# samuelfneumann/RLControl

Hardware: AMD Instinct MI355X
Metric: gradient updates/sec/GPU (batch=100), Pendulum-shaped DDPG (higher is better)
Workload: dtype f32

## Files before the change

rlcontrol_amd/csrc/ddpg_mfma_kernel.h:

```cpp
#pragma once
#include "mfma_blocks.h"
#include "ddpg_rollout_device.h"

namespace {

using namespace mfb;

constexpr int NTW = 2;
constexpr int NT16 = 16;
constexpr int MSTRIDE = mask_stride(NT16);
static_assert(MSTRIDE == 272, "mask stride of the 256-wide kernels");

struct Smem {
    lds_f32* hbuf;
    lds_u8* mask;
    lds_f32* part;
    lds_f32* wvec;
    lds_f32 *x, *x2, *a, *aout, *mu, *dz, *q, *y, *dq;
    lds_f64 *r, *g;
    lds_i64* idx;
    lds_i32* pool;
    lds_i32* dups;
    lds_f32x4* xbuf;
    lds_f32 *w1t, *w1o;
};

__host__ __device__ inline bool rlc_mfma_wide(const RlcDims& d) { return d.S > SMAX || d.A > 2; }

template <bool WIDE = false>
__host__ __device__ inline size_t smem_carve(const RlcDims& d, int MT, lds_u8* base, Smem* out) {
    size_t off = 0;
    auto take = [&](size_t bytes) {
        lds_u8* p = base + off;
        off += (bytes + 15) & ~(size_t)15;
        return p;
    };
    const int MB = MT * 16, A = d.A, LDH = ldh_for(d.H1);
    constexpr bool wide = WIDE;
    const int XL = wide ? xld_for(d.S) : SMAX;
    Smem L;
    L.hbuf = (lds_f32*)take(sizeof(float) * (MB * LDH + 16));
    L.r = (lds_f64*)take(sizeof(double) * MB);
    L.g = (lds_f64*)take(sizeof(double) * MB);
    L.idx = (lds_i64*)take(sizeof(long long) * RLC_MAX_BATCH);
    L.mask = take((size_t)MB * MSTRIDE);
    static_assert(sizeof(float) * kWaves * 6 <= MSTRIDE, "the WIDE form's partials fit the mask rows");
    if constexpr (wide) L.part = (lds_f32*)L.mask;
    else L.part = (lds_f32*)take(sizeof(float) * kWaves * MB * A);
    L.wvec = (lds_f32*)take(sizeof(float) * A * 256);
    L.x = (lds_f32*)take(sizeof(float) * MB * XL);
    L.x2 = (lds_f32*)take(sizeof(float) * MB * XL);
    L.a = (lds_f32*)take(sizeof(float) * MB * A);
    L.aout = (lds_f32*)take(sizeof(float) * MB * A);
    L.mu = (lds_f32*)take(sizeof(float) * MB * A);
    if constexpr (wide) L.dz = L.a;
    else L.dz = (lds_f32*)take(sizeof(float) * MB * A);
    L.q = (lds_f32*)take(sizeof(float) * MB);
    L.y = (lds_f32*)take(sizeof(float) * MB);
    L.dq = (lds_f32*)take(sizeof(float) * MB);
    L.pool = (lds_i32*)take(sizeof(int) * 3 * RLC_MAX_BATCH);
    L.dups = (lds_i32*)take(sizeof(int) * 4);
    if constexpr (wide) {
        auto t13 = [](int n) { return (n + 15) >> 4 == 13; };
        if (t13(d.H1) || t13(d.HA) || t13(d.HC)) L.xbuf = (lds_f32x4*)take(sizeof(float) * 4 * 64 * (MT - (MT + 3) / 4));
        else L.xbuf = nullptr;
    } else {
        L.xbuf = (lds_f32x4*)take(sizeof(float) * 4 * 64 * (MT - (MT + 3) / 4));
    }
    L.w1t = L.w1o = nullptr;
    if (out) *out = L;
    return off;
}

template <int MT, int AD, bool FUSE, bool T4, bool WIDE = false>
__global__ __launch_bounds__(kThreads) void rlc_ddpg_update_mfma_kernel(RlcDev dv, int first_agent, int n_updates,
                                                                        int source, const long long* host_idx,
                                                                        int grad_taps, const RlcRollout* rollout,
                                                                        int q8_first) {
    extern __shared__ __attribute__((aligned(16))) unsigned char smem[];
    using U = Blk<MT, NTW, MSTRIDE, false, false, T4, WIDE>;
    static_assert(WIDE || AD <= 2, "more than two action columns: the WIDE form");
    static_assert(!(WIDE && T4), "the WIDE form has no tail-of-four units");
    constexpr int MB = U::MB;
    const RlcDims d = dv.d;
    U u;
    u.init_geometry();
    u.S = d.S; u.H1 = d.H1; u.B = d.B; u.LDH = ldh_for(d.H1);
    const int XL = WIDE ? xld_for(d.S) : SMAX;
    Smem L;
    smem_carve<WIDE>(d, MT, (lds_u8*)smem, &L);
    u.L.hbuf = L.hbuf; u.L.mask = L.mask; u.L.xbuf = L.xbuf;
    const int tid = u.tid, S = d.S, H1 = d.H1, HA = d.HA, HC = d.HC, B = d.B;
    const int agent = first_agent + blockIdx.x;
    constexpr bool fuse_fwd = FUSE;
    const bool sep = d.sep != 0;

    float* th = dv.theta + (size_t)agent * d.Ppad;
    float* tt = dv.theta_t + (size_t)agent * d.Ppad;
    float* m_a = dv.m_a + (size_t)agent * d.Ppad;
    float* v_a = dv.v_a + (size_t)agent * d.Ppad;
    float* m_c = dv.m_c + (size_t)agent * d.Ppad;
    float* v_c = dv.v_c + (size_t)agent * d.Ppad;
    float* pw = dv.pw + agent * 4;
    const float lr_a = dv.actor_lr[agent], lr_c = dv.critic_lr[agent], tau = dv.tau;
#ifdef RLC_STAMPS
    float* stamp_buf = grad_taps ? dv.tap_gc + (size_t)agent * d.Ppad : nullptr;
    float* tap_gc = nullptr;
    float* tap_ga = nullptr;
#else
    float* tap_gc = grad_taps ? dv.tap_gc + (size_t)agent * d.Ppad : nullptr;
    float* tap_ga = grad_taps ? dv.tap_ga + (size_t)agent * d.Ppad : nullptr;
#endif
    float amax[AD];
#pragma unroll
    for (int j = 0; j < AD; j++) amax[j] = dv.amax[j];

    for (int i = tid; i < MB * AD; i += kThreads) { L.a[i] = 0.f; L.aout[i] = 0.f; L.mu[i] = 0.f; L.dz[i] = 0.f; }
    for (int i = tid; i < MB * XL; i += kThreads) { L.x[i] = 0.f; L.x2[i] = 0.f; }
    for (int i = tid; i < MB; i += kThreads) { L.q[i] = 0.f; L.y[i] = 0.f; L.dq[i] = 0.f; }
    for (int i = tid; i < MB * MSTRIDE / 4; i += kThreads) reinterpret_cast<lds_u32*>(L.mask)[i] = 0u;
    if (tid < 16) L.hbuf[MB * u.LDH + tid] = 0.0f;
    __syncthreads();

    f32x4 acc[MT][NTW];
#ifdef RLC_STAMPS
    long long t_prev = clock64();
    int stamp_i = 0;
#define STAMP()                                                                                  \
    do {                                                                                         \
        if (tid == 0 && stamp_buf) { const long long t = clock64(); stamp_buf[stamp_i] += (float)(t - t_prev); t_prev = t; } \
        stamp_i++;                                                                               \
    } while (0)
    if (stamp_buf) for (int i = tid; i < 64; i += kThreads) stamp_buf[i] = 0.0f;
    const long long t_k0 = clock64(), w_k0 = wall_clock64();
    u.stamp_buf = stamp_buf;
    __syncthreads();
#else
#define STAMP() do {} while (0)
#endif

    for (int upd = 0; upd < n_updates; upd++) {
#ifdef RLC_STAMPS
        stamp_i = 0;
#endif
        asm volatile("" : "+v"(u.c), "+v"(u.g), "+s"(u.wave));
        if (rollout) {
            if (!rlc_train_step_device(rollout, agent, (float*)L.hbuf, upd == 0 ? q8_first : 0)) continue;
        }
        if (!(ablate(4) && upd > 0)) {
        u.sub_begin();
        const RlcRingMeta ring = dv.rep.ring[agent];
        if (source == RLC_SRC_REPLAY_DEVICE_SAMPLER) {
            const unsigned long long call = dv.rep.sample_ctr[agent];
            __syncthreads();
            u.sub_stamp(25);
            rlc_sample_distinct(ring.size, B, dv.rep.seed[agent], call, L.pool, L.idx, L.dups);
            if (tid == 0) dv.rep.sample_ctr[agent] = call + 1;
            u.sub_stamp(26);
        } else if (source == RLC_SRC_REPLAY_HOST_INDICES) {
            for (int b = tid; b < B; b += kThreads) L.idx[b] = host_idx[((size_t)blockIdx.x * n_updates + upd) * B + b];
        }
        __syncthreads();
        for (int b = tid; b < B; b += kThreads) {
            const float *ps, *pa, *ps2;
            if (source == RLC_SRC_STAGING) {
                const size_t slot = (size_t)agent * RLC_MAX_BATCH + b;
                ps = dv.rep.gs + slot * S; pa = dv.rep.ga + slot * AD; ps2 = dv.rep.gs2 + slot * S;
                L.r[b] = dv.rep.gr[slot]; L.g[b] = dv.rep.gg[slot];
            } else {
                const size_t slot = (size_t)agent * dv.rep.cap + ring_slot(ring, dv.rep.cap, L.idx[b]);
                ps = dv.rep.rs + slot * S; pa = dv.rep.ra + slot * AD; ps2 = dv.rep.rs2 + slot * S;
                L.r[b] = dv.rep.rr[slot]; L.g[b] = dv.rep.rg[slot];
            }
            for (int i = 0; i < S; i++) {
                L.x[b * XL + i] = clip_state_val(ps[i], dv.clip_state, dv.smin[i], dv.smax[i]);
                L.x2[b * XL + i] = clip_state_val(ps2[i], dv.clip_state, dv.smin[i], dv.smax[i]);
            }
#pragma unroll
            for (int j = 0; j < AD; j++) L.a[b * AD + j] = pa[j];
        }
        u.sub_stamp(27);
        }
        __syncthreads();
        STAMP();

        u.trunk(tt + d.oW1, tt + d.ob1, L.x2);
        __syncthreads();
        STAMP();
        f32x4 acc2[MT][NTW];
        if constexpr (fuse_fwd) u.fwd_gemm2(acc, acc2, tt + d.oWa2, tt + d.oWc2, HA, H1);
        else u.fwd_gemm(acc, tt + d.oWa2, HA, H1);
        u.template bias_relu<0>(acc, tt + d.oba2, HA);
        u.template row_dot<false, AD>(acc, HA, [&](int n, int j) { return tt[d.oWa3 + n * AD + j]; }, L.part);
        __syncthreads();
        STAMP();
        for (int i = tid; i < B * AD; i += kThreads) {
            const int b = i / AD, j = i % AD;
            L.aout[i] = tanhf(u.template part_sum<AD>(L.part, b, j) + tt[d.oba3 + j]) * amax[j];
        }
        __syncthreads();
        STAMP();
        if constexpr (fuse_fwd) {
#pragma unroll
            for (int mt = 0; mt < MT; mt++)
#pragma unroll
                for (int i = 0; i < NTW; i++) acc[mt][i] = acc2[mt][i];
        } else {
            if (sep) {
                u.trunk(tt + d.oWc1, tt + d.obc1, L.x2);
                __syncthreads();
            }
            u.fwd_gemm(acc, tt + d.oWc2, HC, H1);
        }
        u.template bias_relu<AD>(acc, tt + d.obc2, HC, L.aout, tt + d.oWc2, d.arow0);
        u.template row_dot<false, 1>(acc, HC, [&](int n, int) { return tt[d.oWc3 + n]; }, L.part);
        __syncthreads();
        STAMP();
        for (int b = tid; b < B; b += kThreads) {
            const float qt = u.template part_sum<1>(L.part, b, 0) + tt[d.obc3];
            const float y = (float)(L.r[b] + L.g[b] * (double)qt);
            L.y[b] = y;
            dv.tap_y[(size_t)agent * RLC_MAX_BATCH + b] = y;
        }
        __syncthreads();
        STAMP();

        u.trunk(th + d.oWc1, th + d.obc1, L.x);
        for (int n = tid; n < 256; n += kThreads) L.wvec[n] = n < HC ? th[d.oWc3 + n] : 0.0f;
        __syncthreads();
        STAMP();
        u.fwd_gemm(acc, th + d.oWc2, HC, H1);
        u.template bias_relu<AD>(acc, th + d.obc2, HC, L.a, th + d.oWc2, d.arow0);
        u.template row_dot<false, 1>(acc, HC, [&](int n, int) { return th[d.oWc3 + n]; }, L.part);
        __syncthreads();
        STAMP();
        for (int b = tid; b < B; b += kThreads) {
            const float q = u.template part_sum<1>(L.part, b, 0) + th[d.obc3];
            L.q[b] = q;
            dv.tap_q[(size_t)agent * RLC_MAX_BATCH + b] = q;
            L.dq[b] = 2.0f * (q - L.y[b]) / (float)B;
        }
        __syncthreads();
        STAMP();
        float g_wc3[NTW], g_bc2[NTW];
        {
            const int NT = (HC + 15) >> 4;
#pragma unroll
            for (int i = 0; i < NTW; i++) {
                const int t = u.tile_of(i);
                const int n = 16 * t + u.c;
                const float w3 = (t < NT && n < HC) ? L.wvec[n] : 0.0f;
                float s3 = 0.0f, s2 = 0.0f;
#pragma unroll
                for (int mt = 0; mt < MT; mt++) {
                    const f32x4 dq4 = *reinterpret_cast<const lds_f32x4*>(&L.dq[16 * mt + 4 * u.g]);
#pragma unroll
                    for (int r = 0; r < 4; r++) {
                        const float gv = acc[mt][i][r];
                        s3 += gv * dq4[r];
                        s2 += gv > 0.0f ? dq4[r] * w3 : 0.0f;
                    }
                }
                g_wc3[i] = col4_sum(s3);
                g_bc2[i] = col4_sum(s2);
            }
        }
        u.template store_masks<-2, true>(acc, HC);
        __syncthreads();
        STAMP();
        const float alpha_c = adam_alpha(lr_c, pw[2], pw[3]);
        u.template bwd_gemm<1, -2>(acc, th + d.oWc2, HC, H1, L.dq, L.wvec);
        __syncthreads();
        STAMP();
        u.trunk_grad_adam(acc, th, m_c, v_c, alpha_c, d.oWc1, d.obc1, tap_gc, sep ? tt : nullptr, tau, L.x);
        STAMP();
        u.template wgrad_adam<1, AD, -1>(L.dq, L.a, HC, th + d.oWc2, m_c + d.oWc2, v_c + d.oWc2, alpha_c,
                     tap_gc ? tap_gc + d.oWc2 : nullptr, tt + d.oWc2, tau, L.wvec);
        u.sub_begin();
        {
            const int NT = (HC + 15) >> 4;
#pragma unroll
            for (int i = 0; i < NTW; i++) {
                const int t = u.tile_of(i);
                const int n = 16 * t + u.c;
                if (t < NT && n < HC && u.g < 2) {
                    const int p = (u.g == 0) ? d.oWc3 + n : d.obc2 + n;
                    const float gr = (u.g == 0) ? g_wc3[i] : g_bc2[i];
                    float mm = m_c[p], vv = v_c[p];
                    const float o = tt[p];
                    const float nv = adam_step(th[p], gr, mm, vv, alpha_c);
                    m_c[p] = mm; v_c[p] = vv; th[p] = nv;
                    if (tap_gc) tap_gc[p] = gr;
                    tt[p] = o + tau * (nv - o);
                }
            }
            if (u.wave == 0) {
                float gr = 0.0f;
                for (int b = u.lane; b < MB; b += 64) gr += L.dq[b];
#pragma unroll
                for (int off = 32; off > 0; off >>= 1) gr += __shfl_xor(gr, off, 64);
                if (u.lane == 0) {
                    const int p = d.obc3;
                    float mm = m_c[p], vv = v_c[p];
                    const float o = tt[p];
                    const float nv = adam_step(th[p], gr, mm, vv, alpha_c);
                    m_c[p] = mm; v_c[p] = vv; th[p] = nv;
                    if (tap_gc) tap_gc[p] = gr;
                    tt[p] = o + tau * (nv - o);
                }
            }
        }
        u.sub_stamp(29);
        __syncthreads();
        u.sub_stamp(30);
        STAMP();
        if (tid == 0) { pw[2] *= 0.9f; pw[3] *= 0.999f; }

        u.trunk(th + d.oW1, th + d.ob1, L.x);
        for (int i = tid; i < AD * 256; i += kThreads) {
            const int j = i / 256, n = i % 256;
            L.wvec[i] = n < HA ? th[d.oWa3 + n * AD + j] : 0.0f;
        }
        __syncthreads();
        STAMP();
        f32x4 acc7[MT][NTW];
        if constexpr (fuse_fwd) u.fwd_gemm2(acc, acc7, th + d.oWa2, th + d.oWc2, HA, H1);
        else u.fwd_gemm(acc, th + d.oWa2, HA, H1);
        u.template bias_relu<0>(acc, th + d.oba2, HA);
        u.template row_dot<false, AD>(acc, HA, [&](int n, int j) { return th[d.oWa3 + n * AD + j]; }, L.part);
        if constexpr (!WIDE) u.template store_masks<-2, true>(acc, HA);
        __syncthreads();
        STAMP();
        for (int i = tid; i < B * AD; i += kThreads) {
            const int b = i / AD, j = i % AD;
            const float mu = tanhf(u.template part_sum<AD>(L.part, b, j) + th[d.oba3 + j]);
            L.mu[i] = mu;
            const float ao = mu * amax[j];
            L.aout[i] = ao;
            dv.tap_aout[(size_t)agent * RLC_MAX_BATCH * AD + i] = ao;
        }
        __syncthreads();
        STAMP();
        f32x4 h2acc[MT][NTW];
#pragma unroll
        for (int mt = 0; mt < MT; mt++)
#pragma unroll
            for (int i = 0; i < NTW; i++) h2acc[mt][i] = acc[mt][i];

        if constexpr (fuse_fwd) {
#pragma unroll
            for (int mt = 0; mt < MT; mt++)
#pragma unroll
                for (int i = 0; i < NTW; i++) acc[mt][i] = acc7[mt][i];
        } else {
            if (sep) {
                u.trunk(th + d.oWc1, th + d.obc1, L.x);
                __syncthreads();
            }
            u.fwd_gemm(acc, th + d.oWc2, HC, H1);
        }
        u.template bias_relu<AD>(acc, th + d.obc2, HC, L.aout, th + d.oWc2, d.arow0);
        u.template row_dot<true, AD>(acc, HC, [&](int n, int j) { return th[d.oWc2 + rlc_blk_index(d.arow0 + j, n, HC)] * th[d.oWc3 + n]; },
                                     L.part);
        __syncthreads();
        STAMP();
        for (int i = tid; i < B * AD; i += kThreads) {
            const int b = i / AD, j = i % AD;
            const float dqda = u.template part_sum<AD>(L.part, b, j);
            dv.tap_dqda[(size_t)agent * RLC_MAX_BATCH * AD + i] = dqda;
            const float mu = L.mu[i];
            L.dz[i] = -dqda * (1.0f - mu * mu);
        }
        __syncthreads();
        STAMP();

        if constexpr (WIDE) u.template store_masks<-2, true>(h2acc, HA);
        float g_wa3[NTW][AD], g_ba2[NTW];
        {
            const int NT = (HA + 15) >> 4;
#pragma unroll
            for (int i = 0; i < NTW; i++) {
                const int t = u.tile_of(i);
                const int n = 16 * t + u.c;
                const bool ok = t < NT && n < HA;
                float w3[AD], s3[AD];
#pragma unroll
                for (int j = 0; j < AD; j++) { w3[j] = ok ? L.wvec[j * 256 + n] : 0.0f; s3[j] = 0.0f; }
                float s2 = 0.0f;
#pragma unroll
                for (int mt = 0; mt < MT; mt++)
#pragma unroll
                    for (int r = 0; r < 4; r++) {
                        const int b = 16 * mt + 4 * u.g + r;
                        const float hv = h2acc[mt][i][r];
                        float dd = 0.0f;
#pragma unroll
                        for (int j = 0; j < AD; j++) {
                            const float dzb = L.dz[b * AD + j];
                            s3[j] += hv * dzb;
                            dd += dzb * w3[j];
                        }
                        s2 += hv > 0.0f ? dd : 0.0f;
                    }
#pragma unroll
                for (int j = 0; j < AD; j++) g_wa3[i][j] = col4_sum(s3[j]);
                g_ba2[i] = col4_sum(s2);
            }
        }
        const float alpha_a = adam_alpha(lr_a, pw[0], pw[1]);
        if constexpr (WIDE) __syncthreads();
        u.template bwd_gemm<AD, -2>(acc, th + d.oWa2, HA, H1, L.dz, L.wvec);
        __syncthreads();
        if (sep) {
            u.trunk(th + d.oW1, th + d.ob1, L.x);
            __syncthreads();
        }
        STAMP();
        u.trunk_grad_adam(acc, th, m_a, v_a, alpha_a, d.oW1, d.ob1, tap_ga, tt, tau, L.x);
        STAMP();
        u.template wgrad_adam<AD, 0, -1>(L.dz, nullptr, HA, th + d.oWa2, m_a + d.oWa2, v_a + d.oWa2, alpha_a,
                     tap_ga ? tap_ga + d.oWa2 : nullptr, tt + d.oWa2, tau, L.wvec);
        {
            const int NT = (HA + 15) >> 4;
#pragma unroll
            for (int i = 0; i < NTW; i++) {
                const int t = u.tile_of(i);
                const int n = 16 * t + u.c;
                if constexpr (AD <= 3) {
                    if (t < NT && n < HA && u.g <= AD) {
                        int p = d.oba2 + n;
                        float gr = g_ba2[i];
#pragma unroll
                        for (int j = 0; j < AD; j++)
                            if (u.g == j + 1) { p = d.oWa3 + n * AD + j; gr = g_wa3[i][j]; }
                        float mm = m_a[p], vv = v_a[p];
                        const float o = tt[p];
                        const float nv = adam_step(th[p], gr, mm, vv, alpha_a);
                        m_a[p] = mm; v_a[p] = vv; th[p] = nv;
                        if (tap_ga) tap_ga[p] = gr;
                        tt[p] = o + tau * (nv - o);
                    }
                } else {
                    for (int s = u.g; s <= AD && t < NT && n < HA; s += 4) {
                        int p = d.oba2 + n;
                        float gr = g_ba2[i];
#pragma unroll
                        for (int j = 0; j < AD; j++)
                            if (s == j + 1) { p = d.oWa3 + n * AD + j; gr = g_wa3[i][j]; }
                        float mm = m_a[p], vv = v_a[p];
                        const float o = tt[p];
                        const float nv = adam_step(th[p], gr, mm, vv, alpha_a);
                        m_a[p] = mm; v_a[p] = vv; th[p] = nv;
                        if (tap_ga) tap_ga[p] = gr;
                        tt[p] = o + tau * (nv - o);
                    }
                }
            }
            if (u.wave < AD) {
                const int j = u.wave;
                float gr = 0.0f;
                for (int b = u.lane; b < MB; b += 64) gr += L.dz[b * AD + j];
#pragma unroll
                for (int off = 32; off > 0; off >>= 1) gr += __shfl_xor(gr, off, 64);
                if (u.lane == 0) {
                    const int p = d.oba3 + j;
                    float mm = m_a[p], vv = v_a[p];
                    const float o = tt[p];
                    const float nv = adam_step(th[p], gr, mm, vv, alpha_a);
                    m_a[p] = mm; v_a[p] = vv; th[p] = nv;
                    if (tap_ga) tap_ga[p] = gr;
                    tt[p] = o + tau * (nv - o);
                }
            }
        }
        __syncthreads();
        STAMP();
        if (tid == 0) { pw[0] *= 0.9f; pw[1] *= 0.999f; }
        __syncthreads();
    }
#ifdef RLC_STAMPS
    if (tid == 0 && stamp_buf) {
        stamp_buf[40] = (float)(clock64() - t_k0);
        stamp_buf[41] = (float)(wall_clock64() - w_k0);
    }
#endif
}

template <int MT, int AD, bool FUSE, bool T4, bool WIDE>
int launch_tf(const RlcDev& dv, int first_agent, int n_agents, int n_updates, int source, const long long* idx_dev,
              int grad_taps, hipStream_t st, const RlcRollout* rollout, int q8_first) {
    const size_t lds = smem_carve<WIDE>(dv.d, MT, nullptr, nullptr);
    RLC_REQUIRE(lds <= 160 * 1024, "MFMA DDPG kernel needs %zu B of LDS (> 160 KiB)", lds);
    RLC_REQUIRE(!T4 || rlc_tail4(dv.d.B, MT), "tail-of-four kernel launched for batch %d", dv.d.B);
    RLC_REQUIRE(WIDE == rlc_mfma_wide(dv.d), "state_dim %d / action_dim %d on the %s form of the MFMA kernel", dv.d.S, dv.d.A,
                WIDE ? "wide" : "narrow");
    auto kern = rlc_ddpg_update_mfma_kernel<MT, AD, FUSE, T4, WIDE>;
    static bool attr_set = false;
    if (!attr_set) {
        RLC_HIP(hipFuncSetAttribute((const void*)kern, hipFuncAttributeMaxDynamicSharedMemorySize, 160 * 1024));
        attr_set = true;
    }
    hipLaunchKernelGGL(kern, dim3(n_agents), dim3(kThreads), lds, st, dv, first_agent, n_updates, source, idx_dev,
                       grad_taps, rollout, q8_first);
    RLC_HIP(hipGetLastError());
    return 0;
}

template <int MT, int AD, bool T4, bool WIDE = false>
int launch_t(const RlcDev& dv, int first_agent, int n_agents, int n_updates, int source, const long long* idx_dev,
             int grad_taps, hipStream_t st, const RlcRollout* rollout, int q8_first) {
    if (dv.d.HA == dv.d.HC && !dv.d.sep)
        return launch_tf<MT, AD, true, T4, WIDE>(dv, first_agent, n_agents, n_updates, source, idx_dev, grad_taps, st, rollout, q8_first);
    return launch_tf<MT, AD, false, T4, WIDE>(dv, first_agent, n_agents, n_updates, source, idx_dev, grad_taps, st, rollout, q8_first);
}

}
```

rlcontrol_amd/csrc/mfma_blocks.h:

```cpp
#pragma once
#include <cstdlib>
#include <type_traits>

#include "rlc_common.h"

namespace mfb {

typedef float f32x4 __attribute__((ext_vector_type(4)));

#define RLC_LDS __attribute__((address_space(3)))
typedef RLC_LDS float lds_f32;
typedef RLC_LDS f32x4 lds_f32x4;
typedef RLC_LDS unsigned char lds_u8;
typedef RLC_LDS unsigned int lds_u32;
typedef RLC_LDS int lds_i32;
typedef RLC_LDS double lds_f64;
typedef RLC_LDS long long lds_i64;

#ifndef RLC_ABLATE
#define RLC_ABLATE 0
#endif
constexpr bool ablate(int bit) { return ((RLC_ABLATE) >> bit) & 1; }

constexpr int kThreads = 512;
// ... 274 lines not shown
                for (int s2 = 0; s2 < 4; s2++)
#pragma unroll
                    for (int m = 0; m < NX; m++)
                        accx[m] = XMODE == 2 ? mfma4(da[m][s2], db[s2], accx[m]) : mfma16(da[m][s2], db[s2], accx[m]);
            }
        };
        auto loadA = [&](f32x4 (&dst)[MT], int ch) {
#pragma unroll
            for (int mt = 0; mt < MT; mt++) dst[mt] = *reinterpret_cast<const lds_f32x4*>(arow(mt) + 16 * ch);
        };
        auto loadB = [&](float (&dst)[NOWN][4], int ch) {
#pragma unroll
            for (int i = 0; i < NOWN; i++)
#pragma unroll
                for (int s = 0; s < 4; s++) dst[i][s] = wp[(size_t)ch * wstep + i * tst + 4 * s];
        };
        auto mac = [&](const f32x4 (&a)[MT], const float (&b)[NOWN][4]) {
#pragma unroll
            for (int s = 0; s < 4; s++)
#pragma unroll
                for (int i = 0; i < NOWN; i++)
#pragma unroll
                    for (int mt = 0; mt < MT; mt++) {
                        if (T4 && mt == MT - 1) tq[i] = mfma4(a[mt][s], b[i][s], tq[i]);
                        else acc[mt][i] = mfma16(a[mt][s], b[i][s], acc[mt][i]);
                    }
        };
        loadB(b0, 0);
        loadA(a0, 0);
        loadX(ax0, bx0, 0);
        int ch = 0;
        auto pin = [&]() {
            __builtin_amdgcn_sched_group_barrier(0x020, 4 * NOWN + (XTRA ? 4 : 0), 0);
#pragma unroll
            for (int mt = 0; mt < MT; mt++) {
                __builtin_amdgcn_sched_group_barrier(0x100, 1, 0);
                __builtin_amdgcn_sched_group_barrier(0x008, 4 * NOWN, 0);
            }
            if (XTRA) {
                __builtin_amdgcn_sched_group_barrier(0x100, NX, 0);
                __builtin_amdgcn_sched_group_barrier(0x008, 4 * NX, 0);
            }
        };
        for (; ch + 2 <= KB; ch += 2) {
            loadB(b1, ch + 1);
            loadA(a1, ch + 1);
            loadX(ax1, bx1, ch + 1);
            mac(a0, b0);
            macX(ax0, bx0);
            pin();
            const int nx = ch + 2 < KB ? ch + 2 : KB - 1;
            loadB(b0, nx);
            loadA(a0, nx);
            loadX(ax0, bx0, nx);
            mac(a1, b1);
            macX(ax1, bx1);
            pin();
        }
        if (ch < KB) { mac(a0, b0); macX(ax0, bx0); }
        if (tail8) {
            const int kofs = 16 * KB + 2 * g - 4 * g;
            const int tofs = ((((c >> 2) << 4) + 2 * g) << 2) + (c & 3);
            const float* wt = W + ((size_t)tile0() << 8) + (size_t)KB * wstep + tofs;
            float bt[NOWN][2];
#pragma unroll
            for (int i = 0; i < NOWN; i++)
#pragma unroll
                for (int s2 = 0; s2 < 2; s2++) bt[i][s2] = wt[i * tst + 4 * s2];
            typedef float f32x2 __attribute__((ext_vector_type(2)));
            f32x2 av[MT];
#pragma unroll
            for (int mt = 0; mt < MT; mt++) av[mt] = *reinterpret_cast<const RLC_LDS f32x2*>(arow(mt) + kofs);
#pragma unroll
            for (int s2 = 0; s2 < 2; s2++)
#pragma unroll
                for (int i = 0; i < NOWN; i++)
#pragma unroll
                    for (int mt = 0; mt < MT; mt++) {
                        if (T4 && mt == MT - 1) tq[i] = mfma4(av[mt][s2], bt[i][s2], tq[i]);
                        else acc[mt][i] = mfma16(av[mt][s2], bt[i][s2], acc[mt][i]);
                    }
            if (XTRA) {
                const float* wtx = W + ((size_t)xt << 8) + (size_t)KB * wstep + tofs;
#pragma unroll
                for (int m = 0; m < NX; m++) {
                    const f32x2 avx = *reinterpret_cast<const RLC_LDS f32x2*>(xrow(m) + kofs);
#pragma unroll
                    for (int s2 = 0; s2 < 2; s2++)
                        accx[m] = XMODE == 2 ? mfma4(avx[s2], wtx[4 * s2], accx[m]) : mfma16(avx[s2], wtx[4 * s2], accx[m]);
                }
            }
        }
        if constexpr (T4) {
#pragma unroll
            for (int i = 0; i < NOWN; i++) acc[MT - 1][i] += tail_finish(tq[i]);
            if constexpr (XMODE == 2) accx[0] = tail_finish(accx[0]);
        }
    }

    template <bool ACCUM>
    __device__ __forceinline__ void collect_split(f32x4 (&acc)[MT][NTW], const f32x4 (&accx)[MXS]) {
        if constexpr (NTW >= 2) {
            if (wave >= 5) {
                const int lo = share_lo(wave - 4), hi = share_lo(wave - 3);
#pragma unroll
                for (int m = 0; m < MXS; m++)
                    if (lo + m < hi) L.xbuf[(lo + m - MXS) * 64 + lane] = accx[m];
            }
            __syncthreads();
            if (wave == 4) {
#pragma unroll
                for (int mt = 0; mt < MT; mt++) {
                    f32x4 v;
                    if (mt < MXS) v = accx[mt < MXS ? mt : 0];
                    else v = L.xbuf[(mt - MXS) * 64 + lane];
                    acc[mt][1] = ACCUM ? acc[mt][1] + v : v;
                }
            }
        }
    }

    __device__ __forceinline__ void fwd_gemm(f32x4 (&acc)[MT][NTW], const float* W, int N, int K) {
        const int NT = (N + 15) >> 4;
#pragma unroll
        for (int mt = 0; mt < MT; mt++)
#pragma unroll
            for (int i = 0; i < NTW; i++) acc[mt][i] = f32x4{0.f, 0.f, 0.f, 0.f};
#ifdef RLC_STAMPS
        const long long t_w0 = clock64();
#endif
        if constexpr (ablate(6)) return;
        const int nown = nown_of(NT);
        const bool tail8 = (K & 15) == 8 && K > 16;
        const int KB = tail8 ? K >> 4 : (K + 15) >> 4;
        f32x4 accx[MXS];
        if constexpr (NTW >= 2) {
            if (split_mode(NT)) {
#pragma unroll
                for (int m = 0; m < MXS; m++) accx[m] = f32x4{0.f, 0.f, 0.f, 0.f};
                if (T4 && wave == 7) fwd_loop<1, T4 ? 2 : 1>(acc, W, NT, KB, tail8, accx, NT - 1, share_lo(3));
                else if (wave >= 4) fwd_loop<1, 1>(acc, W, NT, KB, tail8, accx, NT - 1, share_lo(wave - 4));
                else fwd_loop<2, 0>(acc, W, NT, KB, tail8, accx, 0, 0);
                collect_split<false>(acc, accx);
            } else if (nown >= 2) fwd_loop<2, 0>(acc, W, NT, KB, tail8, accx, 0, 0);
            else if (nown == 1) fwd_loop<1, 0>(acc, W, NT, KB, tail8, accx, 0, 0);
        } else {
            if (nown >= 1) fwd_loop<1, 0>(acc, W, NT, KB, tail8, accx, 0, 0);
        }
#ifdef RLC_STAMPS
        if (lane == 0 && stamp_buf) stamp_buf[48 + wave] += (float)(clock64() - t_w0);
#endif
    }

    template <int NOWN, int XMODE>
    __device__ __forceinline__ void fwd_loop2(f32x4 (&accA)[MT][NTW], f32x4 (&accB)[MT][NTW], const float* WA, const float* WB,
                                              int NT, int KB, bool tail8, f32x4 (&accxA)[MXS], f32x4 (&accxB)[MXS], int xt,
                                              int xm0) {
        constexpr bool XTRA = XMODE != 0;
        constexpr int NX = XMODE == 2 ? 1 : MXS;
        const int lofs = ((((c >> 2) << 4) + 4 * g) << 2) + (c & 3);
        const size_t t0 = ((size_t)tile0() << 8) + lofs;
        const float* wpA = WA + t0;
        const float* wpB = WB + t0;
        const int tst = tstep() << 8;
        const size_t wstep = (size_t)NT << 8;
        const lds_f32* ap = L.hbuf + c * LDH + 4 * g;
        const lds_f32* apt = L.hbuf + (TROW + (c & 3)) * LDH + 4 * g;
        auto arow = [&](int mt) { return (T4 && mt == MT - 1) ? apt : ap + 16 * mt * LDH; };
        f32x4 a0[MT], a1[MT];
        float b0[2][NOWN][4], b1[2][NOWN][4];
        f32x4 tqA[NOWN], tqB[NOWN];
#pragma unroll
        for (int i = 0; i < NOWN; i++) { tqA[i] = f32x4{0.f, 0.f, 0.f, 0.f}; tqB[i] = f32x4{0.f, 0.f, 0.f, 0.f}; }
        const size_t tx = ((size_t)xt << 8) + lofs;
        const float* wpxA = WA + tx;
        const float* wpxB = WB + tx;
        const lds_f32* apx = ap + 16 * xm0 * LDH;
        auto xrow = [&](int m) { return XMODE == 2 ? apt : apx + 16 * (xm0 + m < MT ? m : 0) * LDH; };
        f32x4 ax0[NX], ax1[NX];
        float bx0[2][4], bx1[2][4];
        auto loadX = [&](f32x4 (&da)[NX], float (&db)[2][4], int ch) {
            if (XTRA) {
#pragma unroll
                for (int m = 0; m < NX; m++) da[m] = *reinterpret_cast<const lds_f32x4*>(xrow(m) + 16 * ch);
#pragma unroll
                for (int s2 = 0; s2 < 4; s2++) {
                    db[0][s2] = wpxA[(size_t)ch * wstep + 4 * s2];
                    db[1][s2] = wpxB[(size_t)ch * wstep + 4 * s2];
                }
            }
        };
        auto macX = [&](const f32x4 (&da)[NX], const float (&db)[2][4]) {
            if (XTRA) {
#pragma unroll
                for (int s2 = 0; s2 < 4; s2++)
#pragma unroll
                    for (int m = 0; m < NX; m++) {
                        if (XMODE == 2) {
                            accxA[m] = mfma4(da[m][s2], db[0][s2], accxA[m]);
                            accxB[m] = mfma4(da[m][s2], db[1][s2], accxB[m]);
                        } else {
                            accxA[m] = mfma16(da[m][s2], db[0][s2], accxA[m]);
                            accxB[m] = mfma16(da[m][s2], db[1][s2], accxB[m]);
                        }
                    }
            }
        };
        auto loadA = [&](f32x4 (&dst)[MT], int ch) {
#pragma unroll
            for (int mt = 0; mt < MT; mt++) dst[mt] = *reinterpret_cast<const lds_f32x4*>(arow(mt) + 16 * ch);
        };
        auto loadB = [&](float (&dst)[2][NOWN][4], int ch) {
#pragma unroll
            for (int i = 0; i < NOWN; i++)
#pragma unroll
                for (int s = 0; s < 4; s++) {
                    dst[0][i][s] = wpA[(size_t)ch * wstep + i * tst + 4 * s];
                    dst[1][i][s] = wpB[(size_t)ch * wstep + i * tst + 4 * s];
                }
        };
        auto mac = [&](const f32x4 (&a)[MT], const float (&b)[2][NOWN][4]) {
#pragma unroll
            for (int s = 0; s < 4; s++)
#pragma unroll
                for (int i = 0; i < NOWN; i++)
#pragma unroll
                    for (int mt = 0; mt < MT; mt++) {
                        if (T4 && mt == MT - 1) {
                            tqA[i] = mfma4(a[mt][s], b[0][i][s], tqA[i]);
                            tqB[i] = mfma4(a[mt][s], b[1][i][s], tqB[i]);
                        } else {
                            accA[mt][i] = mfma16(a[mt][s], b[0][i][s], accA[mt][i]);
                            accB[mt][i] = mfma16(a[mt][s], b[1][i][s], accB[mt][i]);
                        }
                    }
        };
        loadB(b0, 0);
        loadA(a0, 0);
        loadX(ax0, bx0, 0);
        int ch = 0;
        auto pin = [&]() {
            __builtin_amdgcn_sched_group_barrier(0x020, 8 * NOWN + (XTRA ? 8 : 0), 0);
#pragma unroll
            for (int mt = 0; mt < MT; mt++) {
                __builtin_amdgcn_sched_group_barrier(0x100, 1, 0);
                __builtin_amdgcn_sched_group_barrier(0x008, 8 * NOWN, 0);
            }
            if (XTRA) {
                __builtin_amdgcn_sched_group_barrier(0x100, NX, 0);
                __builtin_amdgcn_sched_group_barrier(0x008, 8 * NX, 0);
            }
        };
        for (; ch + 2 <= KB; ch += 2) {
            loadB(b1, ch + 1);
            loadA(a1, ch + 1);
            loadX(ax1, bx1, ch + 1);
            mac(a0, b0);
            macX(ax0, bx0);
            pin();
            const int nx = ch + 2 < KB ? ch + 2 : KB - 1;
            loadB(b0, nx);
            loadA(a0, nx);
            loadX(ax0, bx0, nx);
            mac(a1, b1);
            macX(ax1, bx1);
            pin();
        }
        if (ch < KB) { mac(a0, b0); macX(ax0, bx0); }
        if (tail8) {
            const int kofs = 16 * KB + 2 * g - 4 * g;
            const int tofs = ((((c >> 2) << 4) + 2 * g) << 2) + (c & 3);
            const size_t tb = ((size_t)tile0() << 8) + (size_t)KB * wstep + tofs;
            float bt[2][NOWN][2];
#pragma unroll
            for (int i = 0; i < NOWN; i++)
#pragma unroll
                for (int s2 = 0; s2 < 2; s2++) {
                    bt[0][i][s2] = WA[tb + i * tst + 4 * s2];
                    bt[1][i][s2] = WB[tb + i * tst + 4 * s2];
                }
            typedef float f32x2 __attribute__((ext_vector_type(2)));
            f32x2 av[MT];
#pragma unroll
            for (int mt = 0; mt < MT; mt++) av[mt] = *reinterpret_cast<const RLC_LDS f32x2*>(arow(mt) + kofs);
#pragma unroll
            for (int s2 = 0; s2 < 2; s2++)
#pragma unroll
                for (int i = 0; i < NOWN; i++)
#pragma unroll
                    for (int mt = 0; mt < MT; mt++) {
                        if (T4 && mt == MT - 1) {
                            tqA[i] = mfma4(av[mt][s2], bt[0][i][s2], tqA[i]);
                            tqB[i] = mfma4(av[mt][s2], bt[1][i][s2], tqB[i]);
                        } else {
                            accA[mt][i] = mfma16(av[mt][s2], bt[0][i][s2], accA[mt][i]);
                            accB[mt][i] = mfma16(av[mt][s2], bt[1][i][s2], accB[mt][i]);
                        }
                    }
            if (XTRA) {
                const size_t txb = ((size_t)xt << 8) + (size_t)KB * wstep + tofs;
#pragma unroll
                for (int m = 0; m < NX; m++) {
                    const f32x2 avx = *reinterpret_cast<const RLC_LDS f32x2*>(xrow(m) + kofs);
#pragma unroll
                    for (int s2 = 0; s2 < 2; s2++) {
                        if (XMODE == 2) {
                            accxA[m] = mfma4(avx[s2], WA[txb + 4 * s2], accxA[m]);
                            accxB[m] = mfma4(avx[s2], WB[txb + 4 * s2], accxB[m]);
                        } else {
                            accxA[m] = mfma16(avx[s2], WA[txb + 4 * s2], accxA[m]);
                            accxB[m] = mfma16(avx[s2], WB[txb + 4 * s2], accxB[m]);
                        }
                    }
                }
            }
        }
        if constexpr (T4) {
#pragma unroll
            for (int i = 0; i < NOWN; i++) {
                accA[MT - 1][i] += tail_finish(tqA[i]);
                accB[MT - 1][i] += tail_finish(tqB[i]);
            }
            if constexpr (XMODE == 2) { accxA[0] = tail_finish(accxA[0]); accxB[0] = tail_finish(accxB[0]); }
        }
    }

    __device__ __forceinline__ void fwd_gemm2(f32x4 (&accA)[MT][NTW], f32x4 (&accB)[MT][NTW], const float* WA, const float* WB,
                                              int N, int K) {
        const int NT = (N + 15) >> 4;
#pragma unroll
        for (int mt = 0; mt < MT; mt++)
#pragma unroll
            for (int i = 0; i < NTW; i++) { accA[mt][i] = f32x4{0.f, 0.f, 0.f, 0.f}; accB[mt][i] = f32x4{0.f, 0.f, 0.f, 0.f}; }
        if constexpr (ablate(6)) return;
        const int nown = nown_of(NT);
        const bool tail8 = (K & 15) == 8 && K > 16;
        const int KB = tail8 ? K >> 4 : (K + 15) >> 4;
        f32x4 accxA[MXS], accxB[MXS];
        if constexpr (NTW >= 2) {
            if (split_mode(NT)) {
#pragma unroll
                for (int m = 0; m < MXS; m++) { accxA[m] = f32x4{0.f, 0.f, 0.f, 0.f}; accxB[m] = f32x4{0.f, 0.f, 0.f, 0.f}; }
                if (T4 && wave == 7) fwd_loop2<1, T4 ? 2 : 1>(accA, accB, WA, WB, NT, KB, tail8, accxA, accxB, NT - 1, share_lo(3));
                else if (wave >= 4) fwd_loop2<1, 1>(accA, accB, WA, WB, NT, KB, tail8, accxA, accxB, NT - 1, share_lo(wave - 4));
                else fwd_loop2<2, 0>(accA, accB, WA, WB, NT, KB, tail8, accxA, accxB, 0, 0);
                collect_split<false>(accA, accxA);
                __syncthreads();
                collect_split<false>(accB, accxB);
            } else if (nown >= 2) fwd_loop2<2, 0>(accA, accB, WA, WB, NT, KB, tail8, accxA, accxB, 0, 0);
            else if (nown == 1) fwd_loop2<1, 0>(accA, accB, WA, WB, NT, KB, tail8, accxA, accxB, 0, 0);
        } else {
            if (nown >= 1) fwd_loop2<1, 0>(accA, accB, WA, WB, NT, KB, tail8, accxA, accxB, 0, 0);
        }
    }

    template <int NE>
    __device__ __forceinline__ void bias_relu(f32x4 (&acc)[MT][NTW], const float* bias, int N, const lds_f32* E = nullptr,
                                              const float* Wx = nullptr ,
                                              int xrow0 = 0) {
        if constexpr (ablate(10)) return;
        const int NT = (N + 15) >> 4;
#pragma unroll
        for (int i = 0; i < NTW; i++) {
            const int t = tile_of(i);
            const int n = 16 * t + c;
            const bool ok = t < NT && n < N;
            const float bs = ok ? bias[n] : 0.0f;
            float wx[NE > 0 ? NE : 1];
#pragma unroll
            for (int j = 0; j < NE; j++) wx[j] = ok ? Wx[rlc_blk_index(xrow0 + j, n, N)] : 0.0f;
#pragma unroll
            for (int mt = 0; mt < MT; mt++)
#pragma unroll
                for (int r = 0; r < 4; r++) {
                    float v = acc[mt][i][r] + bs;
                    if (NE > 0) {
                        const int b = 16 * mt + 4 * g + r;
#pragma unroll
                        for (int j = 0; j < NE; j++) v += E[b * NE + j] * wx[j];
                    }
                    acc[mt][i][r] = ok ? fmaxf(v, 0.0f) : 0.0f;
                }
        }
    }

    template <bool STEP, int NJ, class CF>
    __device__ __forceinline__ void row_dot(const f32x4 (&acc)[MT][NTW], int N, CF cf, lds_f32* part) {
        if constexpr (ablate(8)) return;
        const int NT = (N + 15) >> 4;
        float co[NTW][NJ];
#pragma unroll
        for (int i = 0; i < NTW; i++) {
            const int t = tile_of(i);
            const int n = 16 * t + c;
            const bool ok = t < NT && n < N;
#pragma unroll
            for (int j = 0; j < NJ; j++) co[i][j] = ok ? cf(n, j) : 0.0f;
        }
#pragma unroll
        for (int mt = 0; mt < MT; mt++)
#pragma unroll
            for (int r = 0; r < 4; r++)
#pragma unroll
                for (int j = 0; j < NJ; j++) {
                    float p = 0.0f;
#pragma unroll
                    for (int i = 0; i < NTW; i++) {
                        const float v = acc[mt][i][r];
                        p += STEP ? (v > 0.0f ? co[i][j] : 0.0f) : v * co[i][j];
                    }
                    p = row16_sum(p);
                    if (c == 0) part[((size_t)wave * MB + 16 * mt + 4 * g + r) * NJ + j] = p;
                }
    }

    template <int NJ>
    __device__ __forceinline__ float part_sum(const lds_f32* part, int b, int j) const {
        float s = part[((size_t)0 * MB + b) * NJ + j];
#pragma unroll
        for (int w = 1; w < kWaves; w++) s += part[((size_t)w * MB + b) * NJ + j];
        return s;
    }

    template <int NE>
    __device__ __forceinline__ void concat_head_dots(const f32x4 (&acc)[MT][NTW], const float* bias, int N, const lds_f32* E,
                                                     const float* Wx, int xrow0, const float* w3, lds_f32* part) {
        const int NT = (N + 15) >> 4;
        float bs[NTW], w3n[NTW], wx[NTW][NE];
        bool okk[NTW];
#pragma unroll
        for (int i = 0; i < NTW; i++) {
            const int t = tile_of(i);
            const int n = 16 * t + c;
            const bool ok = t < NT && n < N;
            okk[i] = ok;
            bs[i] = ok ? bias[n] : 0.0f;
            w3n[i] = ok ? w3[n] : 0.0f;
#pragma unroll
            for (int j = 0; j < NE; j++) wx[i][j] = ok ? Wx[rlc_blk_index(xrow0 + j, n, N)] : 0.0f;
        }
#pragma unroll
        for (int mt = 0; mt < MT; mt++)
#pragma unroll
            for (int r = 0; r < 4; r++) {
                const int b = 16 * mt + 4 * g + r;
                float e[NE];
#pragma unroll
                for (int j = 0; j < NE; j++) e[j] = E[b * NE + j];
                float p0 = 0.0f, pj[NE];
#pragma unroll
                for (int j = 0; j < NE; j++) pj[j] = 0.0f;
#pragma unroll
                for (int i = 0; i < NTW; i++) {
                    float v = acc[mt][i][r] + bs[i];
#pragma unroll
                    for (int j = 0; j < NE; j++) v += e[j] * wx[i][j];
                    v = okk[i] ? fmaxf(v, 0.0f) : 0.0f;
                    p0 += v * w3n[i];
#pragma unroll
                    for (int j = 0; j < NE; j++) pj[j] += v > 0.0f ? w3n[i] * wx[i][j] : 0.0f;
                }
                p0 = row16_sum(p0);
#pragma unroll
                for (int j = 0; j < NE; j++) pj[j] = row16_sum(pj[j]);
                if (c == 0) {
                    lds_f32* dst = part + ((size_t)wave * MB + b) * (1 + NE);
                    dst[0] = p0;
#pragma unroll
                    for (int j = 0; j < NE; j++) dst[1 + j] = pj[j];
                }
            }
    }

    template <int BIT, bool OVERWRITE>
    __device__ __forceinline__ void store_masks(const f32x4 (&acc)[MT][NTW], int N) {
        if constexpr (ablate(9)) return;
        const int NT = (N + 15) >> 4;
#pragma unroll
        for (int i = 0; i < NTW; i++) {
            const int t = tile_of(i);
            if (t < NT) {
#pragma unroll
                for (int mt = 0; mt < MT; mt++)
#pragma unroll
                    for (int r = 0; r < 4; r++) {
                        lds_u8* p = &L.mask[(16 * mt + 4 * g + r) * MSTRIDE + 16 * t + c];
                        const unsigned char bit = acc[mt][i][r] > 0.0f ? (unsigned char)(BIT == -2 ? 0x38u : 1u << (BIT < 0 ? 0 : BIT)) : (unsigned char)0;
                        if (OVERWRITE) *p = bit;
                        else *p = (unsigned char)((*p & ~(1u << (BIT < 0 ? 0 : BIT))) | bit);
                    }
            }
        }
    }
// ... 711 lines not shown
```

Baseline: 955,100.

## Pack actor/critic split-tile columns and defer target TD to cut barriers

In the fused actor/critic forward GEMM, when the last N tile is at most half full, the split-mode waves load actor columns 0-7 and critic columns 8-15 into one 16-wide tile. This halves the extra MFMAs and weight loads for that tile, and a DPP row shift then unpacks the critic half. The target-Q partial sums go to a separate LDS buffer so the TD-target reduction can join the online-Q reduction loop, removing two barriers per update. The Adam beta-power update also moves earlier to drop a trailing barrier. This adds LDS use and intricate lane-index logic that is easy to get wrong.

Measured after the change: 978,900 (median of 6 runs). 2.5% higher.

```diff
diff --git a/rlcontrol_amd/csrc/ddpg_mfma_kernel.h b/rlcontrol_amd/csrc/ddpg_mfma_kernel.h
--- a/rlcontrol_amd/csrc/ddpg_mfma_kernel.h
+++ b/rlcontrol_amd/csrc/ddpg_mfma_kernel.h
@@ -22,7 +22,8 @@
     lds_i32* pool;
     lds_i32* dups;
     lds_f32x4* xbuf;
-    lds_f32 *w1t, *w1o;
+    lds_f32* partq;
+    lds_f32* w1o;
 };
 
 __host__ __device__ inline bool rlc_mfma_wide(const RlcDims& d) { return d.S > SMAX || d.A > 2; }
@@ -67,7 +68,9 @@
     } else {
         L.xbuf = (lds_f32x4*)take(sizeof(float) * 4 * 64 * (MT - (MT + 3) / 4));
     }
-    L.w1t = L.w1o = nullptr;
+    if constexpr (wide) L.partq = L.part;
+    else L.partq = (lds_f32*)take(sizeof(float) * kWaves * MB);
+    L.w1o = nullptr;
     if (out) *out = L;
     return off;
 }
@@ -188,7 +191,7 @@
         __syncthreads();
         STAMP();
         f32x4 acc2[MT][NTW];
-        if constexpr (fuse_fwd) u.fwd_gemm2(acc, acc2, tt + d.oWa2, tt + d.oWc2, HA, H1);
+        if constexpr (fuse_fwd) u.template fwd_gemm2<!WIDE>(acc, acc2, tt + d.oWa2, tt + d.oWc2, HA, H1);
         else u.fwd_gemm(acc, tt + d.oWa2, HA, H1);
         u.template bias_relu<0>(acc, tt + d.oba2, HA);
         u.template row_dot<false, AD>(acc, HA, [&](int n, int j) { return tt[d.oWa3 + n * AD + j]; }, L.part);
@@ -213,17 +216,23 @@
             u.fwd_gemm(acc, tt + d.oWc2, HC, H1);
         }
         u.template bias_relu<AD>(acc, tt + d.obc2, HC, L.aout, tt + d.oWc2, d.arow0);
-        u.template row_dot<false, 1>(acc, HC, [&](int n, int) { return tt[d.oWc3 + n]; }, L.part);
-        __syncthreads();
-        STAMP();
-        for (int b = tid; b < B; b += kThreads) {
-            const float qt = u.template part_sum<1>(L.part, b, 0) + tt[d.obc3];
-            const float y = (float)(L.r[b] + L.g[b] * (double)qt);
-            L.y[b] = y;
-            dv.tap_y[(size_t)agent * RLC_MAX_BATCH + b] = y;
-        }
-        __syncthreads();
-        STAMP();
+        u.template row_dot<false, 1>(acc, HC, [&](int n, int) { return tt[d.oWc3 + n]; }, L.partq);
+        constexpr bool td_in_dq = !WIDE && fuse_fwd;
+        if constexpr (!td_in_dq) {
+            __syncthreads();
+            STAMP();
+            for (int b = tid; b < B; b += kThreads) {
+                const float qt = u.template part_sum<1>(L.partq, b, 0) + tt[d.obc3];
+                const float y = (float)(L.r[b] + L.g[b] * (double)qt);
+                L.y[b] = y;
+                dv.tap_y[(size_t)agent * RLC_MAX_BATCH + b] = y;
+            }
+            __syncthreads();
+            STAMP();
+        } else {
+            STAMP();
+            STAMP();
+        }
 
         u.trunk(th + d.oWc1, th + d.obc1, L.x);
         for (int n = tid; n < 256; n += kThreads) L.wvec[n] = n < HC ? th[d.oWc3 + n] : 0.0f;
@@ -235,6 +244,12 @@
         __syncthreads();
         STAMP();
         for (int b = tid; b < B; b += kThreads) {
+            if constexpr (td_in_dq) {
+                const float qt = u.template part_sum<1>(L.partq, b, 0) + tt[d.obc3];
+                const float y = (float)(L.r[b] + L.g[b] * (double)qt);
+                L.y[b] = y;
+                dv.tap_y[(size_t)agent * RLC_MAX_BATCH + b] = y;
+            }
             const float q = u.template part_sum<1>(L.part, b, 0) + th[d.obc3];
             L.q[b] = q;
             dv.tap_q[(size_t)agent * RLC_MAX_BATCH + b] = q;
@@ -324,7 +339,7 @@
         __syncthreads();
         STAMP();
         f32x4 acc7[MT][NTW];
-        if constexpr (fuse_fwd) u.fwd_gemm2(acc, acc7, th + d.oWa2, th + d.oWc2, HA, H1);
+        if constexpr (fuse_fwd) u.template fwd_gemm2<!WIDE>(acc, acc7, th + d.oWa2, th + d.oWc2, HA, H1);
         else u.fwd_gemm(acc, th + d.oWa2, HA, H1);
         u.template bias_relu<0>(acc, th + d.oba2, HA);
         u.template row_dot<false, AD>(acc, HA, [&](int n, int j) { return th[d.oWa3 + n * AD + j]; }, L.part);
@@ -411,6 +426,7 @@
         if constexpr (WIDE) __syncthreads();
         u.template bwd_gemm<AD, -2>(acc, th + d.oWa2, HA, H1, L.dz, L.wvec);
         __syncthreads();
+        if (tid == 0) { pw[0] *= 0.9f; pw[1] *= 0.999f; }
         if (sep) {
             u.trunk(th + d.oW1, th + d.ob1, L.x);
             __syncthreads();
@@ -475,8 +491,6 @@
         }
         __syncthreads();
         STAMP();
-        if (tid == 0) { pw[0] *= 0.9f; pw[1] *= 0.999f; }
-        __syncthreads();
     }
 #ifdef RLC_STAMPS
     if (tid == 0 && stamp_buf) {
diff --git a/rlcontrol_amd/csrc/mfma_blocks.h b/rlcontrol_amd/csrc/mfma_blocks.h
--- a/rlcontrol_amd/csrc/mfma_blocks.h
+++ b/rlcontrol_amd/csrc/mfma_blocks.h
@@ -450,7 +450,7 @@
 #endif
     }
 
-    template <int NOWN, int XMODE>
+    template <int NOWN, int XMODE, bool PACK = false>
     __device__ __forceinline__ void fwd_loop2(f32x4 (&accA)[MT][NTW], f32x4 (&accB)[MT][NTW], const float* WA, const float* WB,
                                               int NT, int KB, bool tail8, f32x4 (&accxA)[MXS], f32x4 (&accxB)[MXS], int xt,
                                               int xm0) {
@@ -470,8 +470,9 @@
         f32x4 tqA[NOWN], tqB[NOWN];
 #pragma unroll
         for (int i = 0; i < NOWN; i++) { tqA[i] = f32x4{0.f, 0.f, 0.f, 0.f}; tqB[i] = f32x4{0.f, 0.f, 0.f, 0.f}; }
-        const size_t tx = ((size_t)xt << 8) + lofs;
-        const float* wpxA = WA + tx;
+        const int cx = PACK ? (c & 7) : c;
+        const size_t tx = ((size_t)xt << 8) + (PACK ? ((((cx >> 2) << 4) + 4 * g) << 2) + (cx & 3) : lofs);
+        const float* wpxA = ((PACK && c >= 8) ? WB : WA) + tx;
         const float* wpxB = WB + tx;
         const lds_f32* apx = ap + 16 * xm0 * LDH;
         auto xrow = [&](int m) { return XMODE == 2 ? apt : apx + 16 * (xm0 + m < MT ? m : 0) * LDH; };
@@ -484,7 +485,7 @@
 #pragma unroll
                 for (int s2 = 0; s2 < 4; s2++) {
                     db[0][s2] = wpxA[(size_t)ch * wstep + 4 * s2];
-                    db[1][s2] = wpxB[(size_t)ch * wstep + 4 * s2];
+                    if constexpr (!PACK) db[1][s2] = wpxB[(size_t)ch * wstep + 4 * s2];
                 }
             }
         };
@@ -496,10 +497,10 @@
                     for (int m = 0; m < NX; m++) {
                         if (XMODE == 2) {
                             accxA[m] = mfma4(da[m][s2], db[0][s2], accxA[m]);
-                            accxB[m] = mfma4(da[m][s2], db[1][s2], accxB[m]);
+                            if constexpr (!PACK) accxB[m] = mfma4(da[m][s2], db[1][s2], accxB[m]);
                         } else {
                             accxA[m] = mfma16(da[m][s2], db[0][s2], accxA[m]);
-                            accxB[m] = mfma16(da[m][s2], db[1][s2], accxB[m]);
+                            if constexpr (!PACK) accxB[m] = mfma16(da[m][s2], db[1][s2], accxB[m]);
                         }
                     }
             }
@@ -538,7 +539,8 @@
         loadX(ax0, bx0, 0);
         int ch = 0;
         auto pin = [&]() {
-            __builtin_amdgcn_sched_group_barrier(0x020, 8 * NOWN + (XTRA ? 8 : 0), 0);
+            constexpr int XB = PACK ? 4 : 8;
+            __builtin_amdgcn_sched_group_barrier(0x020, 8 * NOWN + (XTRA ? XB : 0), 0);
 #pragma unroll
             for (int mt = 0; mt < MT; mt++) {
                 __builtin_amdgcn_sched_group_barrier(0x100, 1, 0);
@@ -546,7 +548,7 @@
             }
             if (XTRA) {
                 __builtin_amdgcn_sched_group_barrier(0x100, NX, 0);
-                __builtin_amdgcn_sched_group_barrier(0x008, 8 * NX, 0);
+                __builtin_amdgcn_sched_group_barrier(0x008, XB * NX, 0);
             }
         };
         for (; ch + 2 <= KB; ch += 2) {
@@ -596,18 +598,19 @@
                         }
                     }
             if (XTRA) {
-                const size_t txb = ((size_t)xt << 8) + (size_t)KB * wstep + tofs;
+                const size_t txb = ((size_t)xt << 8) + (size_t)KB * wstep + (PACK ? ((((cx >> 2) << 4) + 2 * g) << 2) + (cx & 3) : tofs);
+                const float* WXA = (PACK && c >= 8) ? WB : WA;
 #pragma unroll
                 for (int m = 0; m < NX; m++) {
                     const f32x2 avx = *reinterpret_cast<const RLC_LDS f32x2*>(xrow(m) + kofs);
 #pragma unroll
                     for (int s2 = 0; s2 < 2; s2++) {
                         if (XMODE == 2) {
-                            accxA[m] = mfma4(avx[s2], WA[txb + 4 * s2], accxA[m]);
-                            accxB[m] = mfma4(avx[s2], WB[txb + 4 * s2], accxB[m]);
+                            accxA[m] = mfma4(avx[s2], WXA[txb + 4 * s2], accxA[m]);
+                            if constexpr (!PACK) accxB[m] = mfma4(avx[s2], WB[txb + 4 * s2], accxB[m]);
                         } else {
-                            accxA[m] = mfma16(avx[s2], WA[txb + 4 * s2], accxA[m]);
-                            accxB[m] = mfma16(avx[s2], WB[txb + 4 * s2], accxB[m]);
+                            accxA[m] = mfma16(avx[s2], WXA[txb + 4 * s2], accxA[m]);
+                            if constexpr (!PACK) accxB[m] = mfma16(avx[s2], WB[txb + 4 * s2], accxB[m]);
                         }
                     }
                 }
@@ -619,10 +622,14 @@
                 accA[MT - 1][i] += tail_finish(tqA[i]);
                 accB[MT - 1][i] += tail_finish(tqB[i]);
             }
-            if constexpr (XMODE == 2) { accxA[0] = tail_finish(accxA[0]); accxB[0] = tail_finish(accxB[0]); }
-        }
-    }
-
+            if constexpr (XMODE == 2) {
+                accxA[0] = tail_finish(accxA[0]);
+                if constexpr (!PACK) accxB[0] = tail_finish(accxB[0]);
+            }
+        }
+    }
+
+    template <bool PACK = false>
     __device__ __forceinline__ void fwd_gemm2(f32x4 (&accA)[MT][NTW], f32x4 (&accB)[MT][NTW], const float* WA, const float* WB,
                                               int N, int K) {
         const int NT = (N + 15) >> 4;
@@ -636,7 +643,27 @@
         const int KB = tail8 ? K >> 4 : (K + 15) >> 4;
         f32x4 accxA[MXS], accxB[MXS];
         if constexpr (NTW >= 2) {
-            if (split_mode(NT)) {
+            bool packed = false;
+            if constexpr (PACK) packed = split_mode(NT) && ((N - 1) & 15) < 8;
+            if (packed) {
+#pragma unroll
+                for (int m = 0; m < MXS; m++) accxA[m] = f32x4{0.f, 0.f, 0.f, 0.f};
+                if (T4 && wave == 7) fwd_loop2<1, T4 ? 2 : 1, PACK>(accA, accB, WA, WB, NT, KB, tail8, accxA, accxB, NT - 1, share_lo(3));
+                else if (wave >= 4) fwd_loop2<1, 1, PACK>(accA, accB, WA, WB, NT, KB, tail8, accxA, accxB, NT - 1, share_lo(wave - 4));
+                else fwd_loop2<2, 0>(accA, accB, WA, WB, NT, KB, tail8, accxA, accxB, 0, 0);
+                collect_split<false>(accA, accxA);
+                if (wave == 4) {
+#pragma unroll
+                    for (int mt = 0; mt < MT; mt++)
+#pragma unroll
+                        for (int r = 0; r < 4; r++) {
+                            const float v = accA[mt][1][r];
+                            const float o = __int_as_float(__builtin_amdgcn_update_dpp(0, __float_as_int(v), 0x128, 0xf, 0xf, false));
+                            accA[mt][1][r] = c < 8 ? v : 0.0f;
+                            accB[mt][1][r] = c < 8 ? o : 0.0f;
+                        }
+                }
+            } else if (split_mode(NT)) {
 #pragma unroll
                 for (int m = 0; m < MXS; m++) { accxA[m] = f32x4{0.f, 0.f, 0.f, 0.f}; accxB[m] = f32x4{0.f, 0.f, 0.f, 0.f}; }
                 if (T4 && wave == 7) fwd_loop2<1, T4 ? 2 : 1>(accA, accB, WA, WB, NT, KB, tail8, accxA, accxB, NT - 1, share_lo(3));
```
